# yhz0/SQLP

Hardware: AMD Instinct MI355X
Metric: stage-2 subproblems/sec + cut-gen HBM GB/s on STORM (higher is better)
Workload: dtype f64

## Files before the change

### sqlp_amd/csrc/api.hip

```cpp
#include <hip/hip_runtime.h>
#include <algorithm>
#include <cmath>
#include <cstdarg>
#include <cstdio>
#include <cstdlib>
#include <cstring>
#include <string>
#include <vector>
#include <map>
#include <memory>
#include <thread>
#include <chrono>
#include "twosd_internal.h"
#include "twosd_ctx.h"

using namespace twosd;

static thread_local std::string g_err;

int twosd::fail(int code, const char *fmt, ...) {
    char buf[1024];
    va_list ap;
    va_start(ap, fmt);
    vsnprintf(buf, sizeof buf, fmt, ap);
// ... 1784 lines not shown
    const auto t_pe2 = std::chrono::steady_clock::now();
    if (c->CH > 0 && P > 1) {
        if ((rc = upload_big(c, &c->d_kp, kp)) || (rc = upload_big(c, &c->d_ke, ke, kz)) || (rc = upload_big(c, &c->d_kraw, kr, kz)) ||
            (rc = upload_big(c, &c->d_sel_ptr, cap)) || (rc = reserve_selection(c, P, cap[P])))
            return rc;
    }
    c->k_valid = true;
    if (getenv("TWOSD_DEBUG")) {
        auto ms = [](auto a, auto b) { return std::chrono::duration<double, std::milli>(b - a).count(); };
        fprintf(stderr, "prepare_elements P=%d: build %.1f ms, upload ell %.1f ms (%zu entries), selection inputs %.1f ms\n",
                P, ms(t_pe0, t_pe1), ms(t_pe1, t_pe2), ecnt[P], ms(t_pe2, std::chrono::steady_clock::now()));
    }
    return TWOSD_OK;
}

__global__ void pool_xbase_kernel(int P, int MP, const int *__restrict__ brptr, const int *__restrict__ brcol,
                                  const double *__restrict__ brval, const double *__restrict__ b, double *__restrict__ xbase) {
    const size_t t = (size_t)blockIdx.x * blockDim.x + threadIdx.x;
    if (t >= (size_t)P * MP) return;
    const size_t p = t / MP, i = t - p * MP;
    const int *rp = brptr + p * (MP + 1);
    double s = 0.0;
    int q = rp[i];
    const int q1 = rp[i + 1];
    for (; q + 4 <= q1; q += 4) {
        const int c0 = brcol[q], c1 = brcol[q + 1], c2 = brcol[q + 2], c3 = brcol[q + 3];
        const double v0 = brval[q], v1 = brval[q + 1], v2 = brval[q + 2], v3 = brval[q + 3];
        const double b0 = b[c0], b1 = b[c1], b2 = b[c2], b3 = b[c3];
        s = fma(v0, b0, s);
        s = fma(v1, b1, s);
        s = fma(v2, b2, s);
        s = fma(v3, b3, s);
    }
    for (; q < q1; ++q) s = fma(brval[q], b[brcol[q]], s);
    xbase[t] = s;
}

__device__ __forceinline__ double dev_infeas(double x, int bt) {
    const double tol = 1e-9;
    if (bt == BT_Y || bt == BT_L) return x < -tol ? x : 0.0;
    if (bt == BT_G) return x > tol ? x : 0.0;
    return fabs(x) > tol ? x : 0.0;
}

constexpr int kSelStreamThreads = 256;
constexpr double kSelCountWeight = 0.5;
constexpr int kSelStreamRows = 1024;
__global__ void __launch_bounds__(kSelStreamThreads) pool_selstream_kernel(
    int m, int MP, int k, const double *__restrict__ xbase, const int *__restrict__ hb0,
    const int *__restrict__ kp, const int *__restrict__ ke, const double *__restrict__ kraw, const double *__restrict__ xaux,
    int box, int order_rows, float cw, const int *__restrict__ scap, int2 *__restrict__ rec, int *__restrict__ send,
    float *__restrict__ cinf) {
    __shared__ double skey[kSelStreamRows];
    __shared__ int sidx[kSelStreamRows];
    __shared__ int soff[kSelStreamRows];
    __shared__ float cpart[kSelStreamThreads];
    __shared__ int tsum[kSelStreamThreads];
    const int p = blockIdx.x, tid = threadIdx.x;
    const double *coef = xaux + m, *lo_e = xaux + m + k, *hi_e = xaux + m + 2 * k;
    const int *kpp = kp + (size_t)p * (m + 1);
    float cf = 0.0f;
    for (int i = tid; i < kSelStreamRows; i += kSelStreamThreads) {
        double key = INFINITY;
        if (i < m) {
            const int t = (hb0[(size_t)p * MP + i] & 3);
            const double xv = xbase[(size_t)p * MP + i];
            const int q0 = kpp[i], q1 = kpp[i + 1];
            if (q0 == q1) {
                const double f = fabs(dev_infeas(xv, t));
                cf += (float)f + (f > 0.0 ? cw : 0.0f);
            } else {
                double worst = 0.0;
                bool active = true;
                if (box) {
                    double lo = xv, hi = xv, mag = fabs(xv);
                    for (int q = q0; q < q1; ++q) {
                        const int e = ke[q];
                        const double g = coef[e] * kraw[q];
                        const double a = g * lo_e[e], bb = g * hi_e[e];
                        lo += fmin(a, bb);
                        hi += fmax(a, bb);
                        mag += fmax(fabs(a), fabs(bb));
                    }
                    const double tol = 1e-9 + 1e-12 * mag;
                    const bool feasible_box = (t == BT_Y || t == BT_L) ? lo > tol : (t == BT_G) ? hi < -tol : false;
                    if (isfinite(lo) && isfinite(hi) && feasible_box) active = false;
                    worst = (t == BT_Y || t == BT_L) ? -lo : (t == BT_G) ? hi : fmax(fabs(lo), fabs(hi));
                    if (!isfinite(worst)) worst = HUGE_VAL;
                }
                if (active) key = order_rows ? -worst : 0.0;
            }
        }
        skey[i] = key;
        sidx[i] = i;
    }
    cpart[tid] = cf;
    __syncthreads();
    for (int kk = 2; kk <= kSelStreamRows; kk <<= 1) {
        for (int j = kk >> 1; j > 0; j >>= 1) {
            for (int t2 = tid; t2 < kSelStreamRows / 2; t2 += kSelStreamThreads) {
                const int a = 2 * j * (t2 / j) + (t2 % j), b2 = a + j;
                const bool up = (a & kk) == 0;
                const double ka = skey[a], kb = skey[b2];
                const int ia = sidx[a], ib = sidx[b2];
                const bool gt = ka > kb || (ka == kb && ia > ib);
                if (gt == up) {
                    skey[a] = kb; skey[b2] = ka;
                    sidx[a] = ib; sidx[b2] = ia;
                }
            }
            __syncthreads();
        }
    }
    constexpr int PER = kSelStreamRows / kSelStreamThreads;
    int loc[PER], run = 0;
#pragma unroll
    for (int u = 0; u < PER; ++u) {
        const int sp = tid * PER + u;
        const int i = sidx[sp];
        const int c = skey[sp] != INFINITY ? (1 + kpp[i + 1] - kpp[i]) * ((hb0[(size_t)p * MP + i] & 3) == BT_E ? 2 : 1) : 0;
        loc[u] = run;
        run += c;
    }
    tsum[tid] = run;
    __syncthreads();
    if (tid == 0) {
        int acc = 0;
        float cacc = 0.0f;
        for (int t = 0; t < kSelStreamThreads; ++t) {
            const int v = tsum[t];
            tsum[t] = acc;
            acc += v;
            cacc += cpart[t];
        }
        send[p] = scap[p] + acc;
        cinf[p] = cacc;
    }
    __syncthreads();
#pragma unroll
    for (int u = 0; u < PER; ++u) soff[tid * PER + u] = tsum[tid] + loc[u];
    __syncthreads();
    const int lane = tid & 63, wv = tid >> 6;
    const size_t base = (size_t)scap[p];
    for (int sp = wv; sp < kSelStreamRows; sp += kSelStreamThreads / 64) {
        if (skey[sp] == INFINITY) break;
        const int i = sidx[sp];
        const int q0 = kpp[i], q1 = kpp[i + 1];
        int2 *out = rec + base + soff[sp];
        const int t = hb0[(size_t)p * MP + i] & 3;
        const int ncopy = t == BT_E ? 2 : 1;
        for (int cpy = 0; cpy < ncopy; ++cpy) {
            const float sg = (t == BT_Y || t == BT_L || cpy == 1) ? -1.0f : 1.0f;
            int2 *o = out + cpy * (1 + q1 - q0);
            if (lane == 0) o[0] = make_int2(__float_as_int(sg * (float)xbase[(size_t)p * MP + i]), -1);
            for (int q = q0 + lane; q < q1; q += 64) o[1 + q - q0] = make_int2(__float_as_int(sg * (float)kraw[q]), ke[q] * 65 * 8);
        }
    }
}

template <typename T>
static int upload_cap(T **d, size_t *cap, const T *h, size_t n) {
    if (!*d || n > *cap) {
        const size_t nc = std::max<size_t>(n, 1);
        int rc = dalloc(d, nc);
        if (rc) return rc;
        *cap = nc;
    }
    if (n) HIPCHK(hipMemcpy(*d, h, sizeof(T) * n, hipMemcpyHostToDevice));
    return TWOSD_OK;
}

int twosd::prepare_x(twosd_ctx *c, const double *x) {
    const int m = c->L.m, MP = c->MP, k = c->k, n1 = c->n1;
    if (c->prep_valid && c->prep_x.size() == (size_t)n1 && (n1 == 0 || std::equal(c->prep_x.begin(), c->prep_x.end(), x)))
        return TWOSD_OK;
    int rc;
    const auto t_start = std::chrono::steady_clock::now();
    if (!c->k_valid && (rc = prepare_elements(c))) return rc;
    std::vector<double> b;
    rhs_at(c, x, nullptr, b);
    const int P = (int)c->pool.size();
    std::vector<double> coef(std::max(k, 1), 1.0);
    for (int e = 0; e < k; ++e) coef[e] = c->pos_col[e] < 0 ? 1.0 : -x[c->pos_col[e]];
    if (!c->d_xbase || (size_t)P * MP > c->xbase_cap) {
        if ((rc = dalloc(&c->d_xbase, (size_t)P * MP))) return rc;
        c->xbase_cap = (size_t)P * MP;
    }
    if (c->CH > 0) {
        const bool sel = P > 1;
        const bool box = !c->sel_lo.empty();
        std::vector<double> aux((size_t)m + 3 * (size_t)k, 0.0);
        std::copy(b.begin(), b.end(), aux.begin());
        std::copy(coef.begin(), coef.begin() + k, aux.begin() + m);
        if (box) {
            std::copy(c->sel_lo.begin(), c->sel_lo.end(), aux.begin() + m + k);
            std::copy(c->sel_hi.begin(), c->sel_hi.end(), aux.begin() + m + 2 * k);
        }
        if ((rc = upload_cap(&c->d_xaux, &c->xaux_cap, aux.data(), aux.size())) ||
            (rc = upload_cap(&c->d_kcoef, &c->kcoef_cap, coef.data(), coef.size())))
            return rc;
        const size_t tot = (size_t)P * MP;
        hipLaunchKernelGGL(pool_xbase_kernel, dim3((unsigned)((tot + 255) / 256)), dim3(256), 0, c->stream, P, MP, c->d_brptr,
                           c->d_brcol, c->d_brval, c->d_xaux, c->d_xbase);
        HIPCHK(hipGetLastError());
        if (sel) {
            if (MP > kSelStreamRows) return fail(TWOSD_E_UNSUPPORTED, "pool selection: m = %d rows > %d", m, kSelStreamRows);
            double sc = 0.0;
            if (c->has_dist && k > 0) {
                for (int e = 0; e < k; ++e) sc += fabs(coef[e]) * c->dist_mad[e];
                sc /= k;
            }
            c->sel_cw = (float)(kSelCountWeight * sc);
            if (const char *e = getenv("TWOSD_SEL_CW")) c->sel_cw = (float)atof(e);
            static const bool sel_order = !getenv("TWOSD_SEL_ROWORDER") || atoi(getenv("TWOSD_SEL_ROWORDER")) != 0;
            hipLaunchKernelGGL(pool_selstream_kernel, dim3(P), dim3(kSelStreamThreads), 0, c->stream, m, MP, k, c->d_xbase,
                               c->d_hb0, c->d_kp, c->d_ke, c->d_kraw, c->d_xaux, box ? 1 : 0, sel_order ? 1 : 0,
                               c->sel_cw, c->d_sel_ptr, reinterpret_cast<int2 *>(c->d_sel_code), c->d_sel_end, c->d_sel_cinf);
            HIPCHK(hipGetLastError());
        }
        if (getenv("TWOSD_DEBUG") && sel) {
            HIPCHK(hipStreamSynchronize(c->stream));
            std::vector<int> beg(P + 1), end(P);
            HIPCHK(hipMemcpy(beg.data(), c->d_sel_ptr, sizeof(int) * (P + 1), hipMemcpyDeviceToHost));
            HIPCHK(hipMemcpy(end.data(), c->d_sel_end, sizeof(int) * P, hipMemcpyDeviceToHost));
            c->sel_nnz = 0;
            for (int p = 0; p < P; ++p) c->sel_nnz += end[p] - beg[p];
            c->sel_rows = 0;
        }
    }
    c->prep_x.assign(x, x + n1);
    c->prep_valid = true;
    if (getenv("TWOSD_DEBUG")) {
        HIPCHK(hipStreamSynchronize(c->stream));
        fprintf(stderr, "prepare_x: P=%d %.3f ms (%lld selection records)\n", P,
                std::chrono::duration<double, std::milli>(std::chrono::steady_clock::now() - t_start).count(),
                (long long)(c->sel_nnz + c->sel_rows));
    }
    return TWOSD_OK;
}

static int select_pool(twosd_ctx *c, const double *d_dv, int N, int *d_pick, int npool_override) {
    const int P = (int)c->pool.size();
    const bool two = npool_override <= 0 && c->pool_l1 > 0 && c->pool_l1 < P && c->pool_ncand > 0 && (c->d_cand || c->cand_pending);
    const int np1 = npool_override > 0 ? npool_override : two ? c->pool_l1 : P;
    int rc;
    size_t tb = 0, tb2 = 0;
    HIPCHK(sort_by_pool(d_pick, nullptr, N, P, nullptr, &tb, c->stream));
    HIPCHK(sort_by_pool(d_pick, nullptr, N, np1, nullptr, &tb2, c->stream));
    tb = std::max(tb, tb2);
    if ((size_t)N > c->order_cap || tb > c->sort_tmp_bytes) {
        if ((rc = dalloc(&c->d_order, (size_t)N)) || (rc = dalloc(&c->d_sort_tmp, tb))) return rc;
        c->order_cap = N;
        c->sort_tmp_bytes = tb;
    }
    if (two && (size_t)N > c->key_cap) {
        if ((rc = dalloc(&c->d_sel_key, (size_t)N))) return rc;
        c->key_cap = N;
    }
    const int g1 = pool_select_split(N, np1), g2 = two ? pool_refine_split(N, c->pool_ncand) : 1;
    const size_t pneed = (size_t)std::max(g1, g2) * N;
    if (std::max(g1, g2) > 1 && pneed > c->sel_pcap) {
        if ((rc = dalloc(&c->d_sel_pkey, pneed)) || (rc = dalloc(&c->d_sel_ppick, pneed))) return rc;
        c->sel_pcap = pneed;
    }
    PoolSelParams S{};
    S.N = N; S.k = c->k; S.npool = np1; S.dv = d_dv;
    S.kcoef = c->d_kcoef;
    S.cinf = c->d_sel_cinf; S.sptr = c->d_sel_ptr; S.send = c->d_sel_end; S.rec = reinterpret_cast<const int2 *>(c->d_sel_code);
    S.pick = d_pick;
    S.cw = c->sel_cw;
    S.key = two ? c->d_sel_key : nullptr;
    S.pkey = g1 > 1 ? c->d_sel_pkey : nullptr;
    S.ppick = g1 > 1 ? c->d_sel_ppick : nullptr;
    HIPCHK(launch_pool_select(S, c->stream));
    if (two && c->cand_pending &&
        (rc = set_candidates(c, c->cand_pl1, c->cand_pnc, (int)c->cand_p1.size(), c->cand_p1.data(), c->cand_pf.data())))
        return rc;
    if (two) {
        HIPCHK(sort_by_pool(d_pick, c->d_order, N, np1, c->d_sort_tmp, &tb, c->stream));
        PoolRefineParams Q{};
        Q.N = N; Q.k = c->k; Q.ncand = c->pool_ncand; Q.dv = d_dv; Q.kcoef = c->d_kcoef;
        Q.cinf = c->d_sel_cinf; Q.sptr = c->d_sel_ptr; Q.send = c->d_sel_end; Q.rec = S.rec;
        Q.order = c->d_order; Q.cand = c->d_cand; Q.pick = d_pick; Q.key = c->d_sel_key; Q.cw = c->sel_cw;
        Q.pkey = g2 > 1 ? c->d_sel_pkey : nullptr;
        Q.pci = g2 > 1 ? c->d_sel_ppick : nullptr;
        HIPCHK(launch_pool_refine(Q, c->stream));
    }
    HIPCHK(sort_by_pool(d_pick, c->d_order, N, P, c->d_sort_tmp, &tb, c->stream));
    return TWOSD_OK;
}

int twosd::run_lp(twosd_ctx *c, const double *x, const double *d_dv, int N, bool want_pi, bool want_y) {
    LpRun o;
    o.want_pi = want_pi;
    o.want_y = want_y;
    return run_lp_ex(c, x, d_dv, N, o);
}

int twosd::run_lp_ex(twosd_ctx *c, const double *x, const double *d_dv, int N, const LpRun &o) {
    const bool want_pi = o.want_pi, want_y = o.want_y;
    const bool list = o.d_list != nullptr;
    const int NL = list ? o.nlist : N;
    int rc;
    if ((rc = prepare_x(c, x))) return rc;
    if (list && c->pool.size() > 1 && (size_t)N > c->pick_cap) return fail(TWOSD_E_STATE, "LP list mode: no recorded pool picks");
    const int m = c->L.m, n = c->L.n, MP = c->MP, R = c->R;
    if (N > c->out_cap) {
// ... 530 lines not shown
```

### sqlp_amd/csrc/lp_hyper.hip

```cpp
#include <hip/hip_runtime.h>
#include <math.h>
#include <type_traits>
#include "twosd_internal.h"
#include "wave_ops.h"

namespace twosd {

#define HTOL_P 1e-9
#define HTOL_D 1e-9
#define HTOL_PIV 1e-9
#define HPI_ZERO 1e-12


#ifdef TWOSD_STAMPS
#define STAMP_DECL unsigned long long st_acc[10] = {0, 0, 0, 0, 0, 0, 0, 0, 0, 0}; \
    unsigned long long st_last = __builtin_amdgcn_s_memtime();
#define STAMP(i)                                                      \
    {                                                                 \
        const unsigned long long t_ = __builtin_amdgcn_s_memtime();   \
        st_acc[i] += t_ - st_last;                                    \
        st_last = t_;                                                 \
    }
#define STAMP_FLUSH                                                                         \
    if (lane == 0 && P.stamps)                                                              \
// ... 801 lines not shown
                }
#pragma unroll
                for (int o = 32; o > 0; o >>= 1) h += __shfl_xor(h, o);
                keyv = h;
            }
        }
        if constexpr (FULL) {
        if (status == TWOSD_LP_OPTIMAL && (P.pi || P.y)) {
            const double *qc = CP.q;
#pragma unroll
            for (int t = 0; t < R; ++t) {
                const int j = hb[t] >> 2;
                const bool bq = hb[t] >= 0 && j < n;
                const double qj = qc[bq ? j : 0];
                ut[64 * t + lane] = bq ? qj : 0.0;
            }
            h_wave_sync();
            for (int tt = K - 1; tt >= 0; --tt) {
                const int off = etaoff[tt], nnz = etaoff[tt + 1] - off;
                double acc = 0.0;
                for (int e = lane; e < nnz; e += 64) acc = fma(ut[eidx[off + e]], evals[off + e], acc);
                acc = wsum(acc);
                nops += nnz;
                if (lane == 0) ut[etap[tt]] = acc;
                h_wave_sync();
            }
            double pv[R];
            double pmax = 0.0;
#pragma unroll
            for (int t = 0; t < R; ++t) {
                const int cc = 64 * t + lane;
                const int e0 = cc < m ? bcp[cc] : 0, e1 = cc < m ? bcp[cc + 1] : 0;
                double a = 0.0;
#pragma unroll TWOSD_REC_UNROLL
                for (int e = e0; e < e1; ++e) a = fma(ut[P.bci[e]], P.bcv[e], a);
                pv[t] = a;
                pmax = fmax(pmax, fabs(a));
            }
            nops += P.bnnz[pb];
            pmax = wmax(pmax);
            const double zt = HPI_ZERO * (1.0 + pmax);
#pragma unroll
            for (int t = 0; t < R; ++t)
                if (fabs(pv[t]) <= zt) pv[t] = 0.0;
            h_wave_sync();
#pragma unroll
            for (int t = 0; t < R; ++t) ut[64 * t + lane] = 0.0;
            if (P.pi) {
                double *po = P.pi + (size_t)(P.pi_by_pos ? qpos : s) * m;
#pragma unroll
                for (int t = 0; t < R; ++t)
                    if (64 * t + lane < m) po[64 * t + lane] = pv[t];
            }
            if (P.y) {
                double *yo = P.y + (size_t)s * n;
                for (int j = lane; j < n; j += 64) yo[j] = 0.0;
                __builtin_amdgcn_s_waitcnt(0);
                __builtin_amdgcn_wave_barrier();
#pragma unroll
                for (int t = 0; t < R; ++t) {
                    const int j = hb[t] >> 2;
                    if (hb[t] >= 0 && j < n) yo[j] = xB[t];
                }
            }
        } else if (status != TWOSD_LP_OPTIMAL && P.pi) {
            double *po = P.pi + (size_t)(P.pi_by_pos ? qpos : s) * m;
#pragma unroll
            for (int t = 0; t < R; ++t)
                if (64 * t + lane < m) po[64 * t + lane] = NAN;
        }
        if (P.head_out) {
            const size_t ho = (size_t)(P.pi_by_pos ? qpos : s) * m;
#pragma unroll
            for (int t = 0; t < R; ++t)
                if (64 * t + lane < m) P.head_out[ho + 64 * t + lane] = hb[t] >> 2;
        }
        if (P.bkey && status == TWOSD_LP_OPTIMAL) {
            unsigned long long h = 0;
#pragma unroll
            for (int t = 0; t < R; ++t)
                if (64 * t + lane < m) h += mix64((unsigned long long)(hb[t] >> 2));
#pragma unroll
            for (int o = 32; o > 0; o >>= 1) h += __shfl_xor(h, o);
            if (lane == 0) P.bkey[s] = h;
        }
        if (P.eo_K) {
            const int erow = P.pi_by_pos ? qpos : s;
            unsigned long long off64 = 0;
            if (lane == 0 && status == TWOSD_LP_OPTIMAL) off64 = atomicAdd(P.eo_used, (unsigned long long)eoff);
            off64 = __shfl(off64, 0);
            const bool ok = status == TWOSD_LP_OPTIMAL && off64 + (unsigned long long)eoff <= (unsigned long long)P.eo_cap;
            const int off = ok ? (int)off64 : 0;
            if (ok) {
                for (int e = lane; e < eoff; e += 64) {
                    P.eo_eidx[off + e] = eidx[e];
                    P.eo_evals[off + e] = evals[e];
                }
                for (int t = lane; t < K; t += 64) P.eo_etap[(size_t)erow * P.kmax + t] = etap[t];
                for (int t = lane; t <= K; t += 64) P.eo_etaoff[(size_t)erow * (P.kmax + 1) + t] = etaoff[t];
            }
            if (lane == 0) {
                P.eo_K[erow] = ok ? K : -1;
                P.eo_off[erow] = off;
                P.eo_pb[erow] = pb;
            }
        }
        }
        {
            const auto *A = h_args();
            double *const o_obj = A->obj;
            int *const o_status = A->status, *const o_iters = A->iters, *const o_etan = A->etan, *const o_pick = A->pool_pick;
            long long *const o_ops = A->ops;
            unsigned long long *const o_key = A->vkey;
            const int su = __builtin_amdgcn_readfirstlane(s);
            if (lane == 0) {
                o_obj[su] = objv;
                o_status[su] = status;
                o_iters[su] = it;
                if (o_ops) o_ops[su] = (long long)nops;
                if (o_etan) o_etan[su] = eoff;
                if (o_pick) o_pick[su] = pb;
                if (o_key && status == TWOSD_LP_OPTIMAL) o_key[su] = keyv;
            }
        }
        h_wave_sync();
        STAMP(9)
    }
    STAMP_FLUSH
}

__device__ __forceinline__ float h_viol_f(float x, float cw) { return x > 1e-9f ? x + cw : 0.0f; }

constexpr int kSelWaves = 16;
#ifndef TWOSD_SEL_B
#define TWOSD_SEL_B 16
#endif
constexpr int kSelB = TWOSD_SEL_B;
typedef float sel_f2 __attribute__((ext_vector_type(2)));
constexpr int kSelTile = 128;
__device__ __forceinline__ sel_f2 h_viol_f2(sel_f2 x, float cw) {
    sel_f2 r;
    r.x = h_viol_f(x.x, cw);
    r.y = h_viol_f(x.y, cw);
    return r;
}
template <typename RowOf>
__device__ __forceinline__ void h_stage_pairs(float *dvt, const double *__restrict__ dv, const double *__restrict__ kcoef,
                                              int k, int nv, RowOf srow) {
    for (int idx = threadIdx.x; idx < kSelTile * k; idx += 64 * kSelWaves) {
        const int sl = idx / k, e = idx - sl * k;
        dvt[2 * (e * 65 + (sl & 63)) + (sl >> 6)] = sl < nv ? (float)(kcoef[e] * dv[(size_t)srow(sl) * k + e]) : 0.0f;
    }
}
__device__ __forceinline__ const sel_f2 *h_pair_addr(const sel_f2 *dvt2, int off, int lane8) {
    int o;
    asm("v_max_i32 %0, %1, 0" : "=v"(o) : "s"(off));
    return reinterpret_cast<const sel_f2 *>(reinterpret_cast<const char *>(dvt2) + o + lane8);
}
template <typename Alive>
__device__ __forceinline__ sel_f2 h_stream2(const int2 *__restrict__ rec, int j0, int j1, float cinf, float cw,
                                            const sel_f2 *dvt2, int lane, Alive alive2) {
    sel_f2 inf = {cinf, cinf}, x = {0.0f, 0.0f};
    const int lane8 = 8 * lane;
    auto step = [&](int code, float v, sel_f2 dl) {
        if (code < 0) {
            inf += h_viol_f2(x, cw);
            x = (sel_f2){v, v};
        } else {
            x = __builtin_elementwise_fma((sel_f2){v, v}, dl, x);
        }
    };
    int j = (__ballot(alive2(inf)) == 0) ? j1 : j0;
    for (; j + kSelB <= j1; j += kSelB) {
        int2 rc[kSelB];
        sel_f2 dl[kSelB];
#pragma unroll
        for (int u = 0; u < kSelB; ++u) rc[u] = rec[j + u];
#pragma unroll
        for (int u = 0; u < kSelB; ++u) dl[u] = *h_pair_addr(dvt2, rc[u].y, lane8);
#pragma unroll
        for (int u = 0; u < kSelB; ++u) step(rc[u].y, __int_as_float(rc[u].x), dl[u]);
        if (__ballot(alive2(inf)) == 0) return (sel_f2){INFINITY, INFINITY};
    }
    for (; j < j1; ++j) {
        const int2 r = rec[j];
        step(r.y, __int_as_float(r.x), *h_pair_addr(dvt2, r.y, lane8));
    }
    inf += h_viol_f2(x, cw);
    return inf;
}

__global__ void __launch_bounds__(64 * kSelWaves) pool_select_kernel(PoolSelParams S) {
    extern __shared__ float dvt[];
    const sel_f2 *dvt2 = reinterpret_cast<const sel_f2 *>(dvt);
    __shared__ float bsum[kSelWaves][kSelTile];
    __shared__ int bidx[kSelWaves][kSelTile];
    __shared__ unsigned sbest[kSelTile];
    const int lane = threadIdx.x & 63;
    const int wid = __builtin_amdgcn_readfirstlane(threadIdx.x >> 6);
    const int s0 = blockIdx.x * kSelTile;
    const int ns = min(kSelTile, S.N - s0);
    h_stage_pairs(dvt, S.dv, S.kcoef, S.k, ns, [&](int sl) { return s0 + sl; });
    if (threadIdx.x < kSelTile) sbest[threadIdx.x] = 0x7f800000u;
    __syncthreads();
    sel_f2 best = {INFINITY, INFINITY};
    int bpx = 0, bpy = 0;
    auto alive2 = [&](sel_f2 inf) {
        const float ox = __uint_as_float(__hip_atomic_load(&sbest[lane], __ATOMIC_RELAXED, __HIP_MEMORY_SCOPE_WORKGROUP));
        const float oy = __uint_as_float(__hip_atomic_load(&sbest[64 + lane], __ATOMIC_RELAXED, __HIP_MEMORY_SCOPE_WORKGROUP));
        return (inf.x < best.x && inf.x <= ox) || (inf.y < best.y && inf.y <= oy);
    };
    const int p_lo = (int)((long long)S.npool * blockIdx.y / gridDim.y), p_hi = (int)((long long)S.npool * (blockIdx.y + 1) / gridDim.y);
    bpx = bpy = p_lo;
    for (int p = p_lo + wid; p < p_hi; p += kSelWaves) {
        const sel_f2 inf = h_stream2(S.rec, S.sptr[p], S.send[p], S.cinf[p], S.cw, dvt2, lane, alive2);
        if (inf.x < best.x) {
            best.x = inf.x;
            bpx = p;
            atomicMin(&sbest[lane], __float_as_uint(inf.x));
        }
        if (inf.y < best.y) {
            best.y = inf.y;
            bpy = p;
            atomicMin(&sbest[64 + lane], __float_as_uint(inf.y));
        }
    }
    bsum[wid][lane] = best.x; bidx[wid][lane] = bpx;
    bsum[wid][64 + lane] = best.y; bidx[wid][64 + lane] = bpy;
    __syncthreads();
    if (wid < 2) {
        const int sl = 64 * wid + lane;
        if (sl < ns) {
            float b = bsum[0][sl];
            int bp = bidx[0][sl];
            for (int w = 1; w < kSelWaves; ++w) {
                const float v = bsum[w][sl];
                const int pw = bidx[w][sl];
                if (v < b || (v == b && pw < bp)) { b = v; bp = pw; }
            }
            if (gridDim.y == 1) {
                S.pick[s0 + sl] = bp;
                if (S.key) S.key[s0 + sl] = b;
            } else {
                S.ppick[(size_t)blockIdx.y * S.N + s0 + sl] = bp;
                S.pkey[(size_t)blockIdx.y * S.N + s0 + sl] = b;
            }
        }
    }
}

__global__ void __launch_bounds__(64 * kSelWaves) pool_refine_kernel(PoolRefineParams S) {
    extern __shared__ float dvt[];
    const sel_f2 *dvt2 = reinterpret_cast<const sel_f2 *>(dvt);
    __shared__ float rkey[kSelWaves][kSelTile];
    __shared__ int rci[kSelWaves][kSelTile];
    __shared__ unsigned sbest[kSelTile];
    const int lane = threadIdx.x & 63;
    const int wid = __builtin_amdgcn_readfirstlane(threadIdx.x >> 6);
    const int nb = gridDim.x, b = blockIdx.x, xq = nb >> 3, xr = nb & 7, xc = b & 7;
    const int tile = xc * xq + min(xc, xr) + (b >> 3);
    const int t0 = tile * kSelTile;
    const int nv = min(kSelTile, S.N - t0);
    h_stage_pairs(dvt, S.dv, S.kcoef, S.k, nv, [&](int sl) { return S.order[t0 + sl]; });
    const bool vx = lane < nv, vy = 64 + lane < nv;
    const int sx = vx ? S.order[t0 + lane] : 0, sy = vy ? S.order[t0 + 64 + lane] : 0;
    const int px = vx ? S.pick[sx] : -1, py = vy ? S.pick[sy] : -1;
    sel_f2 best = {vx ? S.key[sx] : 0.0f, vy ? S.key[sy] : 0.0f};
    int bcx = -1, bcy = -1;
    if (wid == 0) {
        sbest[lane] = __float_as_uint(best.x);
        sbest[64 + lane] = __float_as_uint(best.y);
    }
    __syncthreads();
    bool mx = false, my = false;
    auto alive2 = [&](sel_f2 inf) {
        const float ox = __uint_as_float(__hip_atomic_load(&sbest[lane], __ATOMIC_RELAXED, __HIP_MEMORY_SCOPE_WORKGROUP));
        const float oy = __uint_as_float(__hip_atomic_load(&sbest[64 + lane], __ATOMIC_RELAXED, __HIP_MEMORY_SCOPE_WORKGROUP));
        return (mx && inf.x < best.x && inf.x <= ox) || (my && inf.y < best.y && inf.y <= oy);
    };
    const int c_lo = (int)((long long)S.ncand * blockIdx.y / gridDim.y), c_hi = (int)((long long)S.ncand * (blockIdx.y + 1) / gridDim.y);
    uint64_t todx = __ballot(vx), tody = __ballot(vy);
    while (todx | tody) {
        const int g = todx ? __builtin_amdgcn_readlane(px, __builtin_ctzll(todx))
                           : __builtin_amdgcn_readlane(py, __builtin_ctzll(tody));
        mx = vx && px == g;
        my = vy && py == g;
        todx &= ~__ballot(mx);
        tody &= ~__ballot(my);
        for (int ci = c_lo + wid; ci < c_hi; ci += kSelWaves) {
            const int cb = S.cand[(size_t)g * S.ncand + ci];
            if (cb < 0) break;
            const sel_f2 inf = h_stream2(S.rec, S.sptr[cb], S.send[cb], S.cinf[cb], S.cw, dvt2, lane, alive2);
            if (mx && inf.x < best.x) {
                best.x = inf.x;
                bcx = ci;
                atomicMin(&sbest[lane], __float_as_uint(inf.x));
            }
            if (my && inf.y < best.y) {
                best.y = inf.y;
                bcy = ci;
                atomicMin(&sbest[64 + lane], __float_as_uint(inf.y));
            }
        }
    }
    rkey[wid][lane] = best.x; rci[wid][lane] = bcx;
    rkey[wid][64 + lane] = best.y; rci[wid][64 + lane] = bcy;
    __syncthreads();
    if (wid < 2) {
        const int sl = 64 * wid + lane;
        if (sl < nv) {
            float bk = rkey[0][sl];
            int bc = rci[0][sl];
            for (int w = 1; w < kSelWaves; ++w) {
                const float v = rkey[w][sl];
                const int cw = rci[w][sl];
                if (v < bk || (v == bk && cw >= 0 && (bc < 0 ? false : cw < bc))) { bk = v; bc = cw; }
            }
            const int s = S.order[t0 + sl];
            if (gridDim.y > 1) {
                S.pkey[(size_t)blockIdx.y * S.N + s] = bk;
                S.pci[(size_t)blockIdx.y * S.N + s] = bc;
            } else if (bc >= 0) {
                S.pick[s] = S.cand[(size_t)S.pick[s] * S.ncand + bc];
            }
        }
    }
}

__global__ void pool_select_merge_kernel(int N, int G, const float *__restrict__ pkey, const int *__restrict__ ppick, int *pick,
                                         float *key) {
    const int s = blockIdx.x * blockDim.x + threadIdx.x;
    if (s >= N) return;
    float b = pkey[s];
    int bp = ppick[s];
    for (int y = 1; y < G; ++y) {
        const float v = pkey[(size_t)y * N + s];
        const int p = ppick[(size_t)y * N + s];
        if (v < b || (v == b && p < bp)) { b = v; bp = p; }
    }
    pick[s] = bp;
    if (key) key[s] = b;
}
__global__ void pool_refine_merge_kernel(int N, int G, int ncand, const float *__restrict__ pkey, const int *__restrict__ pci,
                                         const int *__restrict__ cand, int *pick) {
    const int s = blockIdx.x * blockDim.x + threadIdx.x;
    if (s >= N) return;
    float bk = pkey[s];
    int bc = pci[s];
    for (int y = 1; y < G; ++y) {
        const float v = pkey[(size_t)y * N + s];
        const int c = pci[(size_t)y * N + s];
        if (v < bk || (v == bk && c >= 0 && (bc < 0 ? false : c < bc))) { bk = v; bc = c; }
    }
    if (bc >= 0) pick[s] = cand[(size_t)pick[s] * ncand + bc];
}

static int sel_split(int N, int items) {
    if (getenv("TWOSD_SEL_NOSPLIT")) return 1;
    const int nb = (N + kSelTile - 1) / kSelTile;
    int g = (1024 + nb - 1) / nb;
    g = std::min(g, std::max(1, items / kSelWaves));
    return std::max(1, std::min(g, 64));
}
int pool_select_split(int N, int npool) { return sel_split(N, npool); }
int pool_refine_split(int N, int ncand) { return sel_split(N, ncand); }

hipError_t launch_pool_refine(const PoolRefineParams &p, hipStream_t s) {
    if (p.N <= 0 || p.ncand <= 0) return hipSuccess;
    const int G = p.pkey ? pool_refine_split(p.N, p.ncand) : 1;
    hipLaunchKernelGGL(pool_refine_kernel, dim3((p.N + kSelTile - 1) / kSelTile, G), dim3(64 * kSelWaves), pool_select_lds_bytes(p.k), s, p);
    if (G > 1) hipLaunchKernelGGL(pool_refine_merge_kernel, dim3((p.N + 255) / 256), dim3(256), 0, s, p.N, G, p.ncand, p.pkey, p.pci, p.cand, p.pick);
    return hipGetLastError();
}

size_t pool_select_lds_bytes(int k) { return (size_t)4 * 65 * (kSelTile / 64) * (size_t)std::max(k, 1); }

hipError_t launch_pool_select(const PoolSelParams &p, hipStream_t s) {
    if (p.N <= 0) return hipSuccess;
    const int nb = (p.N + kSelTile - 1) / kSelTile;
    const int G = p.pkey ? pool_select_split(p.N, p.npool) : 1;
    hipLaunchKernelGGL(pool_select_kernel, dim3(nb, G), dim3(64 * kSelWaves), pool_select_lds_bytes(p.k), s, p);
    if (G > 1) hipLaunchKernelGGL(pool_select_merge_kernel, dim3((p.N + 255) / 256), dim3(256), 0, s, p.N, G, p.pkey, p.ppick, p.pick, p.key);
    return hipGetLastError();
}

__global__ void __launch_bounds__(256) queue_records_kernel(int N, const int *__restrict__ order, const int *__restrict__ pick,
                                                           int2 *__restrict__ qrec) {
    const int q = blockIdx.x * blockDim.x + threadIdx.x;
    if (q >= N) return;
    const int s = order ? order[q] : q;
    qrec[q] = make_int2(s, pick ? pick[s] : 0);
}
hipError_t launch_queue_records(const int *order, const int *pick, int2 *qrec, int N, hipStream_t s) {
    if (N <= 0) return hipSuccess;
    hipLaunchKernelGGL(queue_records_kernel, dim3((N + 255) / 256), dim3(256), 0, s, N, order, pick, qrec);
    return hipGetLastError();
}

static const int kHR[] = {1, 2, 4, 9, 16};
static const int kHC[] = {2, 4, 8, 14, 16, 28, 32, 64};

int hyper_rows_per_lane(int m) {
    for (int R : kHR)
        if (m <= 64 * R) return R;
    return -1;
}
int hyper_cols_per_lane(int ncols) {
    for (int C : kHC)
        if (ncols <= 64 * C) return C;
    return -1;
}

template <int R, int C>
static hipError_t hl(const HyperParams &p, int nb, size_t lds, hipStream_t s) {
    if (p.pi || p.y || p.head_out || p.bkey || p.eo_K)
        hipLaunchKernelGGL((lp_hyper_kernel<R, C, true>), dim3(nb), dim3(256), lds, s, p);
    else
        hipLaunchKernelGGL((lp_hyper_kernel<R, C, false>), dim3(nb), dim3(256), lds, s, p);
    return hipGetLastError();
}
template <int R, int C>
static int ho(size_t lds) {
    int nb = 0, nb2 = 0;
    if (hipOccupancyMaxActiveBlocksPerMultiprocessor(&nb, lp_hyper_kernel<R, C, true>, 256, lds) != hipSuccess) return 1;
    if (hipOccupancyMaxActiveBlocksPerMultiprocessor(&nb2, lp_hyper_kernel<R, C, false>, 256, lds) != hipSuccess) return 1;
    nb = std::min(nb, nb2);
    return nb > 0 ? nb : 1;
}

#ifdef HYP_DEV_STORM_ONLY
#define HYPER_C_SWITCH(R, FN, ...)                  \
    switch (C) {                                    \
        case 28: if (R == 9) return FN<9, 28>(__VA_ARGS__); \
    }
#else
#define HYPER_C_SWITCH(R, FN, ...)                  \
    switch (C) {                                    \
        case 2: return FN<R, 2>(__VA_ARGS__);       \
        case 4: return FN<R, 4>(__VA_ARGS__);       \
        case 8: return FN<R, 8>(__VA_ARGS__);       \
        case 14: return FN<R, 14>(__VA_ARGS__);     \
        case 16: return FN<R, 16>(__VA_ARGS__);     \
        case 28: return FN<R, 28>(__VA_ARGS__);     \
        case 32: return FN<R, 32>(__VA_ARGS__);     \
        case 64: return FN<R, 64>(__VA_ARGS__);     \
    }
#endif

hipError_t launch_hyper(int R, int C, const HyperParams &p, int nblocks, size_t lds, hipStream_t s) {
    switch (R) {
        case 1: HYPER_C_SWITCH(1, hl, p, nblocks, lds, s); break;
        case 2: HYPER_C_SWITCH(2, hl, p, nblocks, lds, s); break;
        case 4: HYPER_C_SWITCH(4, hl, p, nblocks, lds, s); break;
        case 9: HYPER_C_SWITCH(9, hl, p, nblocks, lds, s); break;
        case 16: HYPER_C_SWITCH(16, hl, p, nblocks, lds, s); break;
    }
    return hipErrorInvalidValue;
}

int hyper_max_blocks_per_cu(int R, int C, int kmax, int k) {
    const size_t lds = hyper_lds_bytes(R, C, kmax, k);
    switch (R) {
        case 1: HYPER_C_SWITCH(1, ho, lds); break;
        case 2: HYPER_C_SWITCH(2, ho, lds); break;
        case 4: HYPER_C_SWITCH(4, ho, lds); break;
        case 9: HYPER_C_SWITCH(9, ho, lds); break;
        case 16: HYPER_C_SWITCH(16, ho, lds); break;
    }
    return 1;
}

}
```

Before: 16.61 million.

## Use LDS sentinel slot for row-start records to drop per-load clamp

Row-header records now carry a real LDS offset pointing at an extra zeroed sentinel row instead of -1. The per-element v_max clamp in the address computation can then go, and the lane offset is folded into a base pointer. The change also adds a launch-bounds occupancy hint to pool_refine_kernel and drops the XCD-aware tile swizzle. LDS grows by one row, and dropping the swizzle may hurt L2 locality across XCDs.

```diff
diff --git a/sqlp_amd/csrc/api.hip b/sqlp_amd/csrc/api.hip
--- a/sqlp_amd/csrc/api.hip
+++ b/sqlp_amd/csrc/api.hip
@@ -1960,7 +1960,7 @@
         for (int cpy = 0; cpy < ncopy; ++cpy) {
             const float sg = (t == BT_Y || t == BT_L || cpy == 1) ? -1.0f : 1.0f;
             int2 *o = out + cpy * (1 + q1 - q0);
-            if (lane == 0) o[0] = make_int2(__float_as_int(sg * (float)xbase[(size_t)p * MP + i]), -1);
+            if (lane == 0) o[0] = make_int2(__float_as_int(sg * (float)xbase[(size_t)p * MP + i]), k * 65 * 8);
             for (int q = q0 + lane; q < q1; q += 64) o[1 + q - q0] = make_int2(__float_as_int(sg * (float)kraw[q]), ke[q] * 65 * 8);
         }
     }
diff --git a/sqlp_amd/csrc/lp_hyper.hip b/sqlp_amd/csrc/lp_hyper.hip
--- a/sqlp_amd/csrc/lp_hyper.hip
+++ b/sqlp_amd/csrc/lp_hyper.hip
@@ -977,18 +977,20 @@
         dvt[2 * (e * 65 + (sl & 63)) + (sl >> 6)] = sl < nv ? (float)(kcoef[e] * dv[(size_t)srow(sl) * k + e]) : 0.0f;
     }
 }
-__device__ __forceinline__ const sel_f2 *h_pair_addr(const sel_f2 *dvt2, int off, int lane8) {
-    int o;
-    asm("v_max_i32 %0, %1, 0" : "=v"(o) : "s"(off));
-    return reinterpret_cast<const sel_f2 *>(reinterpret_cast<const char *>(dvt2) + o + lane8);
+__device__ __forceinline__ int h_sel_sentinel(int k) { return k * 65 * 8; }
+__device__ __forceinline__ void h_stage_sentinel(float *dvt, int k) {
+    for (int idx = threadIdx.x; idx < 2 * 65; idx += 64 * kSelWaves) dvt[2 * 65 * k + idx] = 0.0f;
+}
+__device__ __forceinline__ const sel_f2 *h_pair_addr(const char *lbase, int off) {
+    return reinterpret_cast<const sel_f2 *>(lbase + off);
 }
 template <typename Alive>
 __device__ __forceinline__ sel_f2 h_stream2(const int2 *__restrict__ rec, int j0, int j1, float cinf, float cw,
-                                            const sel_f2 *dvt2, int lane, Alive alive2) {
+                                            const sel_f2 *dvt2, int sent, int lane, Alive alive2) {
     sel_f2 inf = {cinf, cinf}, x = {0.0f, 0.0f};
-    const int lane8 = 8 * lane;
+    const char *lbase = reinterpret_cast<const char *>(dvt2) + 8 * lane;
     auto step = [&](int code, float v, sel_f2 dl) {
-        if (code < 0) {
+        if (code == sent) {
             inf += h_viol_f2(x, cw);
             x = (sel_f2){v, v};
         } else {
@@ -1002,14 +1004,14 @@
 #pragma unroll
         for (int u = 0; u < kSelB; ++u) rc[u] = rec[j + u];
 #pragma unroll
-        for (int u = 0; u < kSelB; ++u) dl[u] = *h_pair_addr(dvt2, rc[u].y, lane8);
+        for (int u = 0; u < kSelB; ++u) dl[u] = *h_pair_addr(lbase, rc[u].y);
 #pragma unroll
         for (int u = 0; u < kSelB; ++u) step(rc[u].y, __int_as_float(rc[u].x), dl[u]);
         if (__ballot(alive2(inf)) == 0) return (sel_f2){INFINITY, INFINITY};
     }
     for (; j < j1; ++j) {
         const int2 r = rec[j];
-        step(r.y, __int_as_float(r.x), *h_pair_addr(dvt2, r.y, lane8));
+        step(r.y, __int_as_float(r.x), *h_pair_addr(lbase, r.y));
     }
     inf += h_viol_f2(x, cw);
     return inf;
@@ -1025,6 +1027,8 @@
     const int wid = __builtin_amdgcn_readfirstlane(threadIdx.x >> 6);
     const int s0 = blockIdx.x * kSelTile;
     const int ns = min(kSelTile, S.N - s0);
+    const int sent = h_sel_sentinel(S.k);
+    h_stage_sentinel(dvt, S.k);
     h_stage_pairs(dvt, S.dv, S.kcoef, S.k, ns, [&](int sl) { return s0 + sl; });
     if (threadIdx.x < kSelTile) sbest[threadIdx.x] = 0x7f800000u;
     __syncthreads();
@@ -1038,7 +1042,7 @@
     const int p_lo = (int)((long long)S.npool * blockIdx.y / gridDim.y), p_hi = (int)((long long)S.npool * (blockIdx.y + 1) / gridDim.y);
     bpx = bpy = p_lo;
     for (int p = p_lo + wid; p < p_hi; p += kSelWaves) {
-        const sel_f2 inf = h_stream2(S.rec, S.sptr[p], S.send[p], S.cinf[p], S.cw, dvt2, lane, alive2);
+        const sel_f2 inf = h_stream2(S.rec, S.sptr[p], S.send[p], S.cinf[p], S.cw, dvt2, sent, lane, alive2);
         if (inf.x < best.x) {
             best.x = inf.x;
             bpx = p;
@@ -1074,7 +1078,7 @@
     }
 }
 
-__global__ void __launch_bounds__(64 * kSelWaves) pool_refine_kernel(PoolRefineParams S) {
+__global__ void __launch_bounds__(64 * kSelWaves, 8) pool_refine_kernel(PoolRefineParams S) {
     extern __shared__ float dvt[];
     const sel_f2 *dvt2 = reinterpret_cast<const sel_f2 *>(dvt);
     __shared__ float rkey[kSelWaves][kSelTile];
@@ -1082,10 +1086,11 @@
     __shared__ unsigned sbest[kSelTile];
     const int lane = threadIdx.x & 63;
     const int wid = __builtin_amdgcn_readfirstlane(threadIdx.x >> 6);
-    const int nb = gridDim.x, b = blockIdx.x, xq = nb >> 3, xr = nb & 7, xc = b & 7;
-    const int tile = xc * xq + min(xc, xr) + (b >> 3);
+    const int tile = blockIdx.x;
     const int t0 = tile * kSelTile;
     const int nv = min(kSelTile, S.N - t0);
+    const int sent = h_sel_sentinel(S.k);
+    h_stage_sentinel(dvt, S.k);
     h_stage_pairs(dvt, S.dv, S.kcoef, S.k, nv, [&](int sl) { return S.order[t0 + sl]; });
     const bool vx = lane < nv, vy = 64 + lane < nv;
     const int sx = vx ? S.order[t0 + lane] : 0, sy = vy ? S.order[t0 + 64 + lane] : 0;
@@ -1115,7 +1120,7 @@
         for (int ci = c_lo + wid; ci < c_hi; ci += kSelWaves) {
             const int cb = S.cand[(size_t)g * S.ncand + ci];
             if (cb < 0) break;
-            const sel_f2 inf = h_stream2(S.rec, S.sptr[cb], S.send[cb], S.cinf[cb], S.cw, dvt2, lane, alive2);
+            const sel_f2 inf = h_stream2(S.rec, S.sptr[cb], S.send[cb], S.cinf[cb], S.cw, dvt2, sent, lane, alive2);
             if (mx && inf.x < best.x) {
                 best.x = inf.x;
                 bcx = ci;
@@ -1198,7 +1203,7 @@
     return hipGetLastError();
 }
 
-size_t pool_select_lds_bytes(int k) { return (size_t)4 * 65 * (kSelTile / 64) * (size_t)std::max(k, 1); }
+size_t pool_select_lds_bytes(int k) { return (size_t)4 * 65 * (kSelTile / 64) * (size_t)(std::max(k, 0) + 1); }
 
 hipError_t launch_pool_select(const PoolSelParams &p, hipStream_t s) {
     if (p.N <= 0) return hipSuccess;
```

Measured after the change: 17.43 million (median of 6 runs). 4.9% higher.
